# Roia2529/RayTracing-folder

Measured on AMD Instinct MI355X. Metric: Mray/s, higher is better.
Workload: dtype f32

## Files before the change

raytracing_folder_amd/csrc/rt_kernels.hip:

```cpp
#include <hip/hip_runtime.h>
#include <math.h>
#include <string.h>
#include <stdlib.h>
#include <type_traits>
#include "rt_shade.h"

#ifndef RT_WF_GRAB
#define RT_WF_GRAB 2
#endif

#define RT_TRACE_OCC __attribute__((amdgpu_waves_per_eu(TEX ? 2 : 3)))
template <int MODEL, bool TEX, bool FX = false>
RT_TRACE_OCC __global__ __launch_bounds__(RT_BLOCK) void k_primary(ShadeCtx C, PrimaryArgs A)
{
    __shared__ uint32_t s_stack[RT_BVH_STACK * RT_BLOCK];
    const BvhStack stack = bvh_stack(s_stack, RT_BVH_STACK, C.S.bvh_spill);
    Counters cnt = {0, 0, 0, 0, 0};
    uint32_t nprim = 0;
    const uint32_t npix = (A.mode == 1) ? C.W.counts[CNT_PIXLIST] : A.npix;
    const unsigned long long total = (unsigned long long)npix * (unsigned long long)A.ns;
    const unsigned long long stride = (unsigned long long)gridDim.x * blockDim.x;
    __shared__ float s_h2[RT_BLOCK], s_h3[RT_BLOCK];
    const bool h_table = A.mode != 2 && A.ns <= RT_BLOCK;
    if (h_table && (int)threadIdx.x < A.ns) { s_h2[threadIdx.x] = halton(A.j0 + (int)threadIdx.x, 2); s_h3[threadIdx.x] = halton(A.j0 + (int)threadIdx.x, 3); }
    __syncthreads();
    for (unsigned long long base = (unsigned long long)blockIdx.x * blockDim.x; base < total; base += stride) {
        PathIn in;
        const bool active = primary_setup(C, A, base + threadIdx.x, total, h_table, s_h2, s_h3, in);
        if (active) nprim++;
        shade_path<MODEL, TEX, FX>(C, in, active, stack, cnt);
    }
    flush_counters(C.W.stats, cnt, nprim, 0, 0);
}

template <int MODEL, bool TEX, bool FX = false>
RT_TRACE_OCC __global__ __launch_bounds__(RT_BLOCK) void k_bounce(ShadeCtx C, DevRayQueue qin, int level)
{
    __shared__ uint32_t s_stack[RT_BVH_STACK * RT_BLOCK];
    const BvhStack stack = bvh_stack(s_stack, RT_BVH_STACK, C.S.bvh_spill);
    Counters cnt = {0, 0, 0, 0, 0};
    uint32_t nrefl = 0, nrefr = 0;
    uint32_t total = C.W.counts[level];
    if (total > qin.cap) total = qin.cap;
    const uint32_t stride = gridDim.x * blockDim.x;
    for (uint32_t base = blockIdx.x * blockDim.x; base < total; base += stride) {
        const uint32_t gid = base + threadIdx.x;
        const bool active = gid < total;
        PathIn in;
        in.primary = false; in.thr = mk(0, 0, 0); in.absorb = mk(0, 0, 0); in.o = mk(0, 0, 0); in.d = mk(0, 0, 1);
        in.slot = 0; in.bounce = 0; in.kind = 0; in.node = 1; in.sample = 0; in.spec = 0;
        in.side_dir = mk(0, 0, 1); in.side_K = mk(0, 0, 0);
        if (active) {
            const uint32_t src = gid;
            const float4 a = qin.a[src], b = qin.b[src], c = qin.c[src];
            const uint4 dd = qin.d[src];
            in.o = mk(a.x, a.y, a.z); in.d = mk(a.w, b.x, b.y);
            in.thr = mk(b.z, b.w, c.x); in.absorb = mk(c.y, c.z, c.w);
            in.slot = dd.x; in.bounce = (int)(dd.y & 0xFFu); in.kind = (dd.y >> 8) & 0xFFu; in.spec = (dd.y >> 16) & 0xFFu; in.node = dd.z; in.sample = dd.w;
            if (MODEL == RT_SHADE_P6 && in.kind == KIND_REFRACT) {
                const float4 e = qin.e[src];
                in.side_dir = mk(e.x, e.y, e.z); in.side_K = mk(e.w, c.z, c.w);
                in.absorb = mk(c.y, 0, 0);
            }
            if (in.kind == KIND_REFLECT) nrefl++; else nrefr++;
        }
        shade_path<MODEL, TEX, FX>(C, in, active, stack, cnt);
    }
    flush_counters(C.W.stats, cnt, 0, nrefl, nrefr);
}

#ifndef RT_WF_WAVES
#define RT_WF_WAVES 3
#endif
#ifndef RT_WF_TEX_WAVES
#define RT_WF_TEX_WAVES 3
#endif
#define RT_WF_HALTON 64
template <bool TEX> struct WfCfg {
    static constexpr int WAVES = TEX ? RT_WF_TEX_WAVES : RT_WF_WAVES;
#ifndef RT_WF_STACK
#define RT_WF_STACK 928
#endif
    static constexpr int BVH = WAVES >= 3 ? RT_BVH_LDS : RT_BVH_STACK;
    static constexpr int STACK = WAVES >= 3 ? RT_WF_STACK : 1008;
    static constexpr int POP = STACK - 2 * RT_BLOCK + 1 < RT_BLOCK ? STACK - 2 * RT_BLOCK + 1 : RT_BLOCK;
    static_assert(BVH * RT_BLOCK * 4 + STACK * 48 + 2 * RT_WF_HALTON * 4 + 16 <= (WAVES >= 3 ? 53760 : 81920), "LDS budget of the occupancy the kernel is built for");
};
__device__ __forceinline__ uint32_t sample_of_slot(const SlotMap &M, uint32_t slot)
{
    if (M.mode == 2) return M.q0 + slot;
    const uint32_t ql = fastdiv(slot, M.div_ms), j = slot - ql * (uint32_t)M.max_sample;
    DevCamera cam; cam.width = M.width; cam.height = M.height;
    int x = 0, y = 0;
    pixel_of(M.tiles, cam, M.q0 + ql, x, y);
    return ((uint32_t)y * (uint32_t)M.width + (uint32_t)x) * (uint32_t)M.max_sample + j;
}
template <int MODEL, bool TEX, bool FX = false>
__attribute__((amdgpu_waves_per_eu(TEX ? RT_WF_TEX_WAVES : RT_WF_WAVES, TEX ? RT_WF_TEX_WAVES : RT_WF_WAVES))) __global__ __launch_bounds__(RT_BLOCK) void k_wavefront(ShadeCtx C, PrimaryArgs A)
{
    using Cfg = WfCfg<TEX>;
    __shared__ uint32_t s_stack[Cfg::BVH * RT_BLOCK];
    __shared__ float4 s_qa[Cfg::STACK], s_qb[Cfg::STACK], s_qc[Cfg::STACK];
    __shared__ uint32_t s_count, s_batch;
    __shared__ float s_h2[RT_WF_HALTON], s_h3[RT_WF_HALTON];
  if constexpr (RT_WF_PERWAVE && MODEL == RT_SHADE_P12) {
    constexpr int NW = RT_BLOCK / 64;
    constexpr uint32_t STACK_W = (uint32_t)Cfg::STACK / NW;
    constexpr uint32_t POP_W = STACK_W > 128u ? (STACK_W - 127u < 64u ? STACK_W - 127u : 64u) : 1u;
    __shared__ uint32_t s_countw[NW];
    const int wv = (int)(threadIdx.x >> 6), lane = (int)(threadIdx.x & 63);
    float4 *qa = s_qa + wv * STACK_W, *qb = s_qb + wv * STACK_W, *qc = s_qc + wv * STACK_W;
    const BvhStack stack = bvh_stack(s_stack, Cfg::BVH, C.S.bvh_spill);
    Counters cnt = {0, 0, 0, 0, 0};
    uint32_t nprim = 0, nrefl = 0, nrefr = 0;
    const uint32_t npix = (A.mode == 1) ? C.W.counts[CNT_PIXLIST] : A.npix;
    const unsigned long long total = A.mode == 3 ? (unsigned long long)min(*A.qsrc_count, A.qsrc.cap)
                                                 : (unsigned long long)npix * (unsigned long long)A.ns;
    const unsigned long long n_batches = (total + 63ull) / 64ull;
    const bool h_table = A.mode < 2 && A.ns <= RT_WF_HALTON;
    uint32_t *next_batch = C.W.counts + (A.mode == 3 ? CNT_WF2_NEXT : CNT_PRIMARY_NEXT);
    if (h_table && (int)threadIdx.x < A.ns) { s_h2[threadIdx.x] = halton(A.j0 + (int)threadIdx.x, 2); s_h3[threadIdx.x] = halton(A.j0 + (int)threadIdx.x, 3); }
    if (lane == 0) s_countw[wv] = 0;
    C.lds_a = qa; C.lds_b = qb; C.lds_c = qc; C.lds_count = &s_countw[wv]; C.lds_cap = STACK_W;
    __syncthreads();
    (void)s_count; (void)s_batch;
    auto wsync = []() {
        __builtin_amdgcn_fence(__ATOMIC_RELEASE, "wavefront");
        __builtin_amdgcn_wave_barrier();
        __builtin_amdgcn_fence(__ATOMIC_ACQUIRE, "wavefront");
    };
    bool more_primaries = true;
    for (;;) {
        wsync();
        uint32_t waiting = (uint32_t)__builtin_amdgcn_readfirstlane((int)s_countw[wv]);
        if (waiting > STACK_W) waiting = STACK_W;
        const bool pop = waiting >= POP_W || (!more_primaries && waiting > 0);
        if (!pop && !more_primaries) break;
        PathIn in;
        bool active;
        if (pop) {
            const uint32_t n = min(waiting, 64u);
            active = (uint32_t)lane < n;
            in.primary = false; in.thr = mk(0, 0, 0); in.absorb = mk(0, 0, 0); in.o = mk(0, 0, 0); in.d = mk(0, 0, 1);
            in.slot = 0; in.bounce = 0; in.kind = 0; in.node = 1; in.sample = 0; in.spec = 0;
            in.side_dir = mk(0, 0, 1); in.side_K = mk(0, 0, 0);
            if (active) {
                const uint32_t src = waiting - 1u - (uint32_t)lane;
                const float4 a = qa[src], b = qb[src], c = qc[src];
                in.o = mk(a.x, a.y, a.z); in.d = mk(a.w, b.x, b.y);
                in.thr = mk(b.z, b.w, c.x);
                in.slot = __float_as_uint(c.y);
                const uint32_t pk = __float_as_uint(c.z);
                in.bounce = (int)(pk & 0xFu); in.kind = (pk >> 4) & 0xFu; in.spec = (pk >> 8) & 0xFFu; in.node = __float_as_uint(c.w);
                const float *ab = C.S.materials[pk >> 16].absorption;
                in.absorb = (MODEL == RT_SHADE_FIN) ? ld3(ab) : mk(ab[0], 0, 0);
                if (C.S.stochastic || MODEL == RT_SHADE_P12) in.sample = sample_of_slot(C.sm, in.slot);
                if (in.kind == KIND_REFLECT) nrefl++; else nrefr++;
            }
            wsync();
            if (lane == 0) s_countw[wv] = waiting - n;
        } else {
            uint32_t bt = 0;
            if (lane == 0) { bt = atomicAdd(next_batch, 1u); if (s_countw[wv] > STACK_W) s_countw[wv] = STACK_W; }
            const unsigned long long batch = (uint32_t)__builtin_amdgcn_readfirstlane((int)bt);
            if (batch >= n_batches) { more_primaries = false; continue; }
            if (A.mode == 3) {
                const unsigned long long src = batch * 64ull + (unsigned)lane;
                active = src < total;
                in.primary = false; in.thr = mk(0, 0, 0); in.absorb = mk(0, 0, 0); in.o = mk(0, 0, 0); in.d = mk(0, 0, 1);
                in.slot = 0; in.bounce = 0; in.kind = 0; in.node = 1; in.sample = 0; in.spec = 0;
                in.side_dir = mk(0, 0, 1); in.side_K = mk(0, 0, 0);
                if (active) {
                    const float4 a = A.qsrc.a[src], b = A.qsrc.b[src], c = A.qsrc.c[src];
                    const uint4 dd = A.qsrc.d[src];
                    in.o = mk(a.x, a.y, a.z); in.d = mk(a.w, b.x, b.y);
                    in.thr = mk(b.z, b.w, c.x); in.absorb = mk(c.y, c.z, c.w);
                    in.slot = dd.x; in.bounce = (int)(dd.y & 0xFFu); in.kind = (dd.y >> 8) & 0xFFu; in.spec = (dd.y >> 16) & 0xFFu; in.node = dd.z; in.sample = dd.w;
                    if (in.kind == KIND_REFLECT) nrefl++; else nrefr++;
                }
            } else {
                active = primary_setup(C, A, batch * 64ull + (unsigned)lane, total, h_table, s_h2, s_h3, in);
                if (active) nprim++;
            }
        }
        wsync();
        shade_path<MODEL, TEX, FX>(C, in, active, stack, cnt);
    }
    flush_counters(C.W.stats, cnt, nprim, nrefl, nrefr);
  } else {
    const BvhStack stack = bvh_stack(s_stack, Cfg::BVH, C.S.bvh_spill);
    Counters cnt = {0, 0, 0, 0, 0};
    uint32_t nprim = 0, nrefl = 0, nrefr = 0;
    const uint32_t npix = (A.mode == 1) ? C.W.counts[CNT_PIXLIST] : A.npix;
    const unsigned long long total = A.mode == 3 ? (unsigned long long)min(*A.qsrc_count, A.qsrc.cap)
                                                 : (unsigned long long)npix * (unsigned long long)A.ns;
    const unsigned long long n_batches = (total + RT_BLOCK - 1) / RT_BLOCK;
    const bool h_table = A.mode < 2 && A.ns <= RT_WF_HALTON;
    uint32_t *next_batch = C.W.counts + (A.mode == 3 ? CNT_WF2_NEXT : CNT_PRIMARY_NEXT);
    if (h_table && (int)threadIdx.x < A.ns) { s_h2[threadIdx.x] = halton(A.j0 + (int)threadIdx.x, 2); s_h3[threadIdx.x] = halton(A.j0 + (int)threadIdx.x, 3); }
    if (threadIdx.x == 0) s_count = 0;
    C.lds_a = s_qa; C.lds_b = s_qb; C.lds_c = s_qc; C.lds_count = &s_count; C.lds_cap = (A.lds_rays && A.lds_rays < (uint32_t)Cfg::STACK) ? A.lds_rays : (uint32_t)Cfg::STACK;
    bool more_primaries = true;
    const uint32_t grab = n_batches >= 128ull * gridDim.x ? (uint32_t)RT_WF_GRAB : 1u;
    unsigned long long grabbed = 0; uint32_t in_hand = 0;
    for (;;) {
        __syncthreads();
        const uint32_t packed = s_count;
        const uint32_t w0 = packed & 0xFFFFu, w1 = packed >> 16;
        const uint32_t pside = w1 > w0 ? 1u : 0u;
        const uint32_t waiting = w0 + w1;
        const bool pop = waiting >= (uint32_t)Cfg::POP || (!more_primaries && waiting > 0);
        if (!pop && !more_primaries) break;
        __syncthreads();
        PathIn in;
        bool active;
        if (pop) {
            const uint32_t wside = pside ? w1 : w0;
            const uint32_t n = min(wside, (uint32_t)RT_BLOCK);
            active = threadIdx.x < n;
            in.primary = false; in.thr = mk(0, 0, 0); in.absorb = mk(0, 0, 0); in.o = mk(0, 0, 0); in.d = mk(0, 0, 1);
            in.slot = 0; in.bounce = 0; in.kind = 0; in.node = 1; in.sample = 0; in.spec = 0;
            in.side_dir = mk(0, 0, 1); in.side_K = mk(0, 0, 0);
            if (active) {
                const uint32_t src = pside ? C.lds_cap - wside + threadIdx.x : wside - 1u - threadIdx.x;
                const float4 a = s_qa[src], b = s_qb[src], c = s_qc[src];
                in.o = mk(a.x, a.y, a.z); in.d = mk(a.w, b.x, b.y);
                in.thr = mk(b.z, b.w, c.x);
                in.slot = __float_as_uint(c.y);
                const uint32_t pk = __float_as_uint(c.z);
                in.bounce = (int)(pk & 0xFu); in.kind = (pk >> 4) & 0xFu; in.spec = (pk >> 8) & 0xFFu; in.node = __float_as_uint(c.w);
                const float *ab = C.S.materials[pk >> 16].absorption;
                in.absorb = (MODEL == RT_SHADE_FIN) ? ld3(ab) : mk(ab[0], 0, 0);
                if (C.S.stochastic || MODEL == RT_SHADE_P12) in.sample = sample_of_slot(C.sm, in.slot);
                if (in.kind == KIND_REFLECT) nrefl++; else nrefr++;
            }
            __syncthreads();
            if (threadIdx.x == 0) s_count = packed - (n << (16u * pside));
        } else {
            if (in_hand == 0) {
                if (threadIdx.x == 0) s_batch = atomicAdd(next_batch, 1u);
                __syncthreads();
                grabbed = (unsigned long long)s_batch * grab;
                in_hand = grab;
            }
            const unsigned long long batch = grabbed + (grab - in_hand);
            in_hand--;
            if (batch >= n_batches) { more_primaries = false; continue; }
            if (A.mode == 3) {
                const unsigned long long src = batch * RT_BLOCK + threadIdx.x;
                active = src < total;
                in.primary = false; in.thr = mk(0, 0, 0); in.absorb = mk(0, 0, 0); in.o = mk(0, 0, 0); in.d = mk(0, 0, 1);
                in.slot = 0; in.bounce = 0; in.kind = 0; in.node = 1; in.sample = 0; in.spec = 0;
                in.side_dir = mk(0, 0, 1); in.side_K = mk(0, 0, 0);
                if (active) {
                    const float4 a = A.qsrc.a[src], b = A.qsrc.b[src], c = A.qsrc.c[src];
                    const uint4 dd = A.qsrc.d[src];
                    in.o = mk(a.x, a.y, a.z); in.d = mk(a.w, b.x, b.y);
                    in.thr = mk(b.z, b.w, c.x); in.absorb = mk(c.y, c.z, c.w);
                    in.slot = dd.x; in.bounce = (int)(dd.y & 0xFFu); in.kind = (dd.y >> 8) & 0xFFu; in.spec = (dd.y >> 16) & 0xFFu; in.node = dd.z; in.sample = dd.w;
                    if (in.kind == KIND_REFLECT) nrefl++; else nrefr++;
                }
            } else {
                active = primary_setup(C, A, batch * RT_BLOCK + threadIdx.x, total, h_table, s_h2, s_h3, in);
                if (active) nprim++;
            }
        }
        __syncthreads();
        shade_path<MODEL, TEX, FX>(C, in, active, stack, cnt);
    }
    flush_counters(C.W.stats, cnt, nprim, nrefl, nrefr);
  }
}

struct FeatureArgs {
    DevCamera cam; DevTiles tiles;
    uint32_t q0, npix;
    int min_sample, max_sample;
    FastDiv div_ms;
    const uint8_t *second;
    int by_walk;
    float *normal, *albedo, *alpha; int32_t *object_id;
};

__global__ __launch_bounds__(256) void k_mark_second(DevWork W, uint8_t *second, uint32_t npix)
{
    const uint32_t n = W.counts[CNT_PIXLIST];
    for (uint32_t i = blockIdx.x * blockDim.x + threadIdx.x; i < n; i += gridDim.x * blockDim.x) {
        const uint32_t ql = W.pixel_list[i];
        if (ql < npix) second[ql] = 1;
    }
}

template <int MODEL, bool TEX>
__attribute__((amdgpu_waves_per_eu(TEX ? 3 : 4, TEX ? 3 : 4))) __global__ __launch_bounds__(RT_BLOCK) void k_features(ShadeCtx C, FeatureArgs F)
{
    __shared__ uint32_t s_stack[RT_BVH_STACK * RT_BLOCK];
    const BvhStack stack = bvh_stack(s_stack, RT_BVH_STACK, C.S.bvh_spill);
    Counters cnt = {0, 0, 0, 0, 0};
    PrimaryArgs A;
    A.cam = F.cam; A.tiles = F.tiles; A.q0 = F.q0; A.npix = F.npix; A.j0 = 0; A.ns = F.max_sample; A.max_sample = F.max_sample; A.mode = 0;
    A.rays = nullptr; A.div_ns = F.div_ms; A.lds_rays = 0; A.qsrc_count = nullptr;
    const unsigned long long total = (unsigned long long)F.npix * (unsigned long long)F.max_sample;
    __shared__ float s_h2[RT_BLOCK], s_h3[RT_BLOCK];
    const bool h_table = F.max_sample <= RT_BLOCK;
    if (h_table && (int)threadIdx.x < F.max_sample) { s_h2[threadIdx.x] = halton((int)threadIdx.x, 2); s_h3[threadIdx.x] = halton((int)threadIdx.x, 3); }
    __syncthreads();
    const bool need_trace = F.normal != nullptr || F.albedo != nullptr || F.object_id != nullptr;
    for (uint32_t ql = blockIdx.x * blockDim.x + threadIdx.x; ql < F.npix; ql += gridDim.x * blockDim.x) {
        int x = 0, y = 0;
        if (!pixel_of(F.tiles, F.cam, F.q0 + ql, x, y)) continue;
        const int ns = F.second[ql] ? F.max_sample : F.min_sample;
        const uint8_t *hitf = C.W.sample_hit + (size_t)ql * F.max_sample;
        int n = 0;
        for (int j = 0; j < ns; j++) n += hitf[j] ? 1 : 0;
        V3 nrm = mk(0, 0, 0), alb = mk(0, 0, 0);
        int id = -1;
        if (n > 0 && need_trace) {
            const float inv = 1 / (float)n;
            for (int j = 0; j < ns; j++) {
                if (!hitf[j]) continue;
                PathIn in;
                if (!primary_setup(C, A, (unsigned long long)ql * (unsigned)F.max_sample + (unsigned)j, total, h_table, s_h2, s_h3, in)) continue;
                Hit h;
                if (!trace<false, MODEL, TEX>(C.S, in.o, in.d, BIGFLOAT, h, stack, cnt)) continue;
                nrm = nrm + h.N * inv;
                if (F.albedo) {
                    V3 kd, ks;
                    material_colors<TEX>(C.S, h, C.S.materials[C.S.node_material[h.node]], kd, ks);
                    alb = alb + kd * inv;
                }
                id = h.node;
            }
        }
        const size_t o = F.by_walk ? (size_t)F.q0 + ql : (size_t)y * F.cam.width + x;
        if (F.normal) { F.normal[3 * o] = nrm.x; F.normal[3 * o + 1] = nrm.y; F.normal[3 * o + 2] = nrm.z; }
        if (F.albedo) { F.albedo[3 * o] = alb.x; F.albedo[3 * o + 1] = alb.y; F.albedo[3 * o + 2] = alb.z; }
        if (F.alpha) F.alpha[o] = (float)n / (float)ns;
        if (F.object_id) F.object_id[o] = id;
    }
}

static bool env_is(const char *name, const char *value) { const char *e = getenv(name); return e && !strcmp(e, value); }
static bool env_wavefront() { static const bool on = !env_is("RT_TRACER", "levels"); return on; }
static bool env_p12_wavefront() { static const bool on = !env_is("RT_P12_TRACER", "levels"); return on; }
static bool env_queue_pass() { static const bool on = !(getenv("RT_WF_QUEUE_PASS") && getenv("RT_WF_QUEUE_PASS")[0] == '0'); return on; }
static uint32_t env_lds_rays()
{
    const char *e = getenv("RT_WF_LDS_RAYS");
    const long v = e ? atol(e) : 0;
    return v > 0 ? (uint32_t)v : 0u;
}

static bool scene_textured(const DevScene &S) { return S.material_maps != nullptr || S.env_map.texture != RT_MAP_NONE; }

bool rtk_wavefront_usable(const DevScene &S, const rt_params &P)
{
    const bool wavefront = env_wavefront(), p12 = env_p12_wavefront();
    const bool model_ok = P.shade_model == RT_SHADE_FIN || P.shade_model == RT_SHADE_P13 ||
                          (P.shade_model == RT_SHADE_P12 && p12 && P.hemisphere_sample <= 2);
    if (!wavefront || !model_ok) return false;
    return S.max_bvh_depth <= (scene_textured(S) ? WfCfg<true>::BVH : WfCfg<false>::BVH) + (S.max_bvh_depth > RT_BVH_LDS ? RT_BVH_SPILL : 0);
}
static int wavefront_blocks(const DevScene &S) { return 256 * (scene_textured(S) ? RT_WF_TEX_WAVES : RT_WF_WAVES); }

static ShadeCtx make_ctx(const DevScene &S, const DevWork &W, const rt_params &P)
{
    ShadeCtx C = {};
    C.S = S; C.S.bvh_spill = W.bvh_spill; C.W = W; C.P = P;
    return C;
}
static ShadeCtx make_ctx(const DevScene &S, const DevWork &W, const rt_params &P, int level, unsigned long long *fx)
{
    ShadeCtx C = make_ctx(S, W, P);
    C.qout = W.rq[level & 1]; C.qout_count = W.counts + level; C.fx = fx;
    return C;
}
static SlotMap make_slotmap(const RenderPass &pass, const DevTiles &tiles_prepared)
{
    SlotMap m; m.tiles = tiles_prepared; m.width = pass.cam.width; m.height = pass.cam.height; m.q0 = pass.q0; m.max_sample = pass.max_sample; m.mode = pass.mode;
    m.div_ms = fastdiv_make((uint32_t)(pass.max_sample > 0 ? pass.max_sample : 1));
    return m;
}

template <int M> using Model = std::integral_constant<int, M>;
template <bool HAS_FX, int M, class F>
static void dispatch_flags(bool tex, bool fx, F &launch)
{
    if constexpr (HAS_FX) {
        if (fx) { if (tex) launch(Model<M>{}, std::true_type{}, std::true_type{}); else launch(Model<M>{}, std::false_type{}, std::true_type{}); return; }
    }
    if (tex) launch(Model<M>{}, std::true_type{}, std::false_type{}); else launch(Model<M>{}, std::false_type{}, std::false_type{});
}
template <bool HAS_FX, int FALLBACK, int... MODELS, class F>
static void dispatch(int model, bool tex, bool fx, F &&launch)
{
    const bool found = ((model == MODELS ? (dispatch_flags<HAS_FX, MODELS>(tex, fx, launch), true) : false) || ...);
    if (!found) dispatch_flags<HAS_FX, FALLBACK>(tex, fx, launch);
}
static void launch_wavefront(hipStream_t st, int grid, const ShadeCtx &C, const PrimaryArgs &A)
{
    dispatch<true, RT_SHADE_P13, RT_SHADE_FIN, RT_SHADE_P12>(C.P.shade_model, scene_textured(C.S), C.fx != nullptr, [&](auto m, auto tex, auto fx) {
        hipLaunchKernelGGL((k_wavefront<m(), tex(), fx()>), dim3(grid), dim3(RT_BLOCK), 0, st, C, A);
    });
}

void rtk_launch_primary(hipStream_t st, const DevScene &S, const DevWork &W, const rt_params &P, const RenderPass &pass, int max_blocks)
{
    ShadeCtx C = make_ctx(S, W, P, 1, pass.fx);
    PrimaryArgs A; A.cam = pass.cam; A.tiles = pass.tiles; A.q0 = pass.q0; A.npix = pass.npix; A.j0 = pass.j0; A.ns = pass.ns;
    A.max_sample = pass.max_sample; A.mode = pass.mode; A.rays = pass.rays; A.lds_rays = env_lds_rays();
    tiles_prepare(A.tiles);
    A.div_ns = fastdiv_make((uint32_t)(pass.ns > 0 ? pass.ns : 1));
    C.sm = make_slotmap(pass, A.tiles);
    const unsigned long long samples = (unsigned long long)pass.npix * pass.ns;
    if (rtk_wavefront_usable(S, P)) { launch_wavefront(st, grid_for(samples, RT_BLOCK, wavefront_blocks(S)), C, A); return; }
    const int grid = grid_for(samples, RT_BLOCK, max_blocks);
    dispatch<true, RT_SHADE_FIN, RT_SHADE_P13, RT_SHADE_P12, RT_SHADE_P6, RT_SHADE_P3>(P.shade_model, scene_textured(S), pass.fx != nullptr, [&](auto m, auto tex, auto fx) {
        hipLaunchKernelGGL((k_primary<m(), tex(), fx()>), dim3(grid), dim3(RT_BLOCK), 0, st, C, A);
    });
}

bool rtk_launch_wavefront_queue(hipStream_t st, const DevScene &S, const DevWork &W, const rt_params &P, const RenderPass &pass)
{
    if (!env_queue_pass() || !rtk_wavefront_usable(S, P)) return false;
    ShadeCtx C = make_ctx(S, W, P, 2, pass.fx);
    DevTiles tp = pass.tiles;
    tiles_prepare(tp);
    C.sm = make_slotmap(pass, tp);
    PrimaryArgs A;
    memset(&A, 0, sizeof A);
    A.mode = 3; A.ns = 1; A.qsrc = W.rq[1]; A.qsrc_count = W.counts + 1; A.lds_rays = env_lds_rays();
    A.div_ns = fastdiv_make(1u);
    launch_wavefront(st, wavefront_blocks(S), C, A);
    return true;
}

void rtk_launch_bounce(hipStream_t st, const DevScene &S, const DevWork &W, const rt_params &P, int level, int max_blocks, unsigned long long *fx)
{
    if (P.shade_model == RT_SHADE_P3) return;
    const ShadeCtx C = make_ctx(S, W, P, level + 1, fx);
    const DevRayQueue &qin = W.rq[level & 1];
    dispatch<true, RT_SHADE_FIN, RT_SHADE_P13, RT_SHADE_P12, RT_SHADE_P6>(P.shade_model, scene_textured(S), fx != nullptr, [&](auto m, auto tex, auto fx_) {
        hipLaunchKernelGGL((k_bounce<m(), tex(), fx_()>), dim3(max_blocks), dim3(RT_BLOCK), 0, st, C, qin, level);
    });
}

void rtk_launch_features(hipStream_t st, const DevScene &S, const DevWork &W, const rt_params &P, const RenderPass &pass,
                         uint8_t *second, const DevFeatures &out, bool by_walk)
{
    const uint32_t npix = pass.npix;
    if (npix == 0) return;
    (void)hipMemsetAsync(second, 0, npix, st);
    if (P.max_sample > P.min_sample) hipLaunchKernelGGL(k_mark_second, dim3(grid_for(npix, 256, 1024)), dim3(256), 0, st, W, second, npix);
    const ShadeCtx C = make_ctx(S, W, P);
    FeatureArgs F; F.cam = pass.cam; F.tiles = pass.tiles; F.q0 = pass.q0; F.npix = npix; F.min_sample = P.min_sample; F.max_sample = P.max_sample;
    tiles_prepare(F.tiles);
    F.div_ms = fastdiv_make((uint32_t)(P.max_sample > 0 ? P.max_sample : 1));
    F.second = second; F.by_walk = by_walk ? 1 : 0;
    F.normal = out.normal; F.albedo = out.albedo; F.alpha = out.alpha; F.object_id = out.object_id;
    const int grid = grid_for(npix, RT_BLOCK, RT_TRACE_BLOCKS);
    dispatch<false, RT_SHADE_FIN, RT_SHADE_P13, RT_SHADE_P12, RT_SHADE_P6, RT_SHADE_P3>(P.shade_model, scene_textured(S), false, [&](auto m, auto tex, auto) {
        hipLaunchKernelGGL((k_features<m(), tex()>), dim3(grid), dim3(RT_BLOCK), 0, st, C, F);
    });
}
```

Before: 9192.

## Run streaks of primary batches without re-syncing when the secondary queue is quiet

The wavefront loop now processes several grabbed primary batches back to back inside one outer iteration when few secondary rays were pushed since the last check, provided the LDS queue has headroom. The aim is to skip the per-iteration __syncthreads and queue-state polling that happen between every primary batch. Some barrier placement is also changed, since the pop path now syncs after updating the count and the fetch path syncs unconditionally. The cost is that secondary rays can sit in LDS longer, and the headroom heuristic must keep the queue from overflowing during a streak.

```diff
diff --git a/raytracing_folder_amd/csrc/rt_kernels.hip b/raytracing_folder_amd/csrc/rt_kernels.hip
--- a/raytracing_folder_amd/csrc/rt_kernels.hip
+++ b/raytracing_folder_amd/csrc/rt_kernels.hip
@@ -7,6 +7,9 @@
 
 #ifndef RT_WF_GRAB
 #define RT_WF_GRAB 2
+#endif
+#ifndef RT_WF_STREAK_QUIET
+#define RT_WF_STREAK_QUIET (2 * RT_BLOCK)
 #endif
 
 #define RT_TRACE_OCC __attribute__((amdgpu_waves_per_eu(TEX ? 2 : 3)))
@@ -203,6 +206,7 @@
     bool more_primaries = true;
     const uint32_t grab = n_batches >= 128ull * gridDim.x ? (uint32_t)RT_WF_GRAB : 1u;
     unsigned long long grabbed = 0; uint32_t in_hand = 0;
+    uint32_t settled = 0;
     for (;;) {
         __syncthreads();
         const uint32_t packed = s_count;
@@ -211,13 +215,14 @@
         const uint32_t waiting = w0 + w1;
         const bool pop = waiting >= (uint32_t)Cfg::POP || (!more_primaries && waiting > 0);
         if (!pop && !more_primaries) break;
-        __syncthreads();
+        const uint32_t pushed = waiting - settled;
         PathIn in;
-        bool active;
+        bool active = false;
+        uint32_t n = 1;
         if (pop) {
             const uint32_t wside = pside ? w1 : w0;
-            const uint32_t n = min(wside, (uint32_t)RT_BLOCK);
-            active = threadIdx.x < n;
+            const uint32_t np = min(wside, (uint32_t)RT_BLOCK);
+            active = threadIdx.x < np;
             in.primary = false; in.thr = mk(0, 0, 0); in.absorb = mk(0, 0, 0); in.o = mk(0, 0, 0); in.d = mk(0, 0, 1);
             in.slot = 0; in.bounce = 0; in.kind = 0; in.node = 1; in.sample = 0; in.spec = 0;
             in.side_dir = mk(0, 0, 1); in.side_K = mk(0, 0, 0);
@@ -235,38 +240,44 @@
                 if (in.kind == KIND_REFLECT) nrefl++; else nrefr++;
             }
             __syncthreads();
-            if (threadIdx.x == 0) s_count = packed - (n << (16u * pside));
+            if (threadIdx.x == 0) s_count = packed - (np << (16u * pside));
+            settled = waiting - np;
+            __syncthreads();
         } else {
-            if (in_hand == 0) {
-                if (threadIdx.x == 0) s_batch = atomicAdd(next_batch, 1u);
-                __syncthreads();
-                grabbed = (unsigned long long)s_batch * grab;
-                in_hand = grab;
-            }
-            const unsigned long long batch = grabbed + (grab - in_hand);
-            in_hand--;
-            if (batch >= n_batches) { more_primaries = false; continue; }
-            if (A.mode == 3) {
-                const unsigned long long src = batch * RT_BLOCK + threadIdx.x;
-                active = src < total;
-                in.primary = false; in.thr = mk(0, 0, 0); in.absorb = mk(0, 0, 0); in.o = mk(0, 0, 0); in.d = mk(0, 0, 1);
-                in.slot = 0; in.bounce = 0; in.kind = 0; in.node = 1; in.sample = 0; in.spec = 0;
-                in.side_dir = mk(0, 0, 1); in.side_K = mk(0, 0, 0);
-                if (active) {
-                    const float4 a = A.qsrc.a[src], b = A.qsrc.b[src], c = A.qsrc.c[src];
-                    const uint4 dd = A.qsrc.d[src];
-                    in.o = mk(a.x, a.y, a.z); in.d = mk(a.w, b.x, b.y);
-                    in.thr = mk(b.z, b.w, c.x); in.absorb = mk(c.y, c.z, c.w);
-                    in.slot = dd.x; in.bounce = (int)(dd.y & 0xFFu); in.kind = (dd.y >> 8) & 0xFFu; in.spec = (dd.y >> 16) & 0xFFu; in.node = dd.z; in.sample = dd.w;
-                    if (in.kind == KIND_REFLECT) nrefl++; else nrefr++;
+            const bool fetch = in_hand == 0;
+            if (fetch && threadIdx.x == 0) s_batch = atomicAdd(next_batch, 1u);
+            __syncthreads();
+            if (fetch) { grabbed = (unsigned long long)s_batch * grab; in_hand = grab; }
+            if (pushed <= (uint32_t)RT_WF_STREAK_QUIET)
+                while (n < in_hand && waiting + n * (uint32_t)RT_WF_STREAK_QUIET + 2u * RT_BLOCK <= C.lds_cap) n++;
+            settled = waiting;
+        }
+        for (uint32_t k = 0; k < n; k++) {
+            if (!pop) {
+                const unsigned long long batch = grabbed + (grab - in_hand);
+                in_hand--;
+                if (batch >= n_batches) { more_primaries = false; break; }
+                if (A.mode == 3) {
+                    const unsigned long long src = batch * RT_BLOCK + threadIdx.x;
+                    active = src < total;
+                    in.primary = false; in.thr = mk(0, 0, 0); in.absorb = mk(0, 0, 0); in.o = mk(0, 0, 0); in.d = mk(0, 0, 1);
+                    in.slot = 0; in.bounce = 0; in.kind = 0; in.node = 1; in.sample = 0; in.spec = 0;
+                    in.side_dir = mk(0, 0, 1); in.side_K = mk(0, 0, 0);
+                    if (active) {
+                        const float4 a = A.qsrc.a[src], b = A.qsrc.b[src], c = A.qsrc.c[src];
+                        const uint4 dd = A.qsrc.d[src];
+                        in.o = mk(a.x, a.y, a.z); in.d = mk(a.w, b.x, b.y);
+                        in.thr = mk(b.z, b.w, c.x); in.absorb = mk(c.y, c.z, c.w);
+                        in.slot = dd.x; in.bounce = (int)(dd.y & 0xFFu); in.kind = (dd.y >> 8) & 0xFFu; in.spec = (dd.y >> 16) & 0xFFu; in.node = dd.z; in.sample = dd.w;
+                        if (in.kind == KIND_REFLECT) nrefl++; else nrefr++;
+                    }
+                } else {
+                    active = primary_setup(C, A, batch * RT_BLOCK + threadIdx.x, total, h_table, s_h2, s_h3, in);
+                    if (active) nprim++;
                 }
-            } else {
-                active = primary_setup(C, A, batch * RT_BLOCK + threadIdx.x, total, h_table, s_h2, s_h3, in);
-                if (active) nprim++;
-            }
+            }
+            shade_path<MODEL, TEX, FX>(C, in, active, stack, cnt);
         }
-        __syncthreads();
-        shade_path<MODEL, TEX, FX>(C, in, active, stack, cnt);
     }
     flush_counters(C.W.stats, cnt, nprim, nrefl, nrefr);
   }
```

Measured after the change: 9189. No clear change (-0.0%).
